# DorianaG01/trajectory_generation

Measured on AMD Instinct MI355X. Metric: MPC steps/sec (batch=4096, N=20), higher is better.
Workload: dtype f64

## Files before the change

### trajectory_generation_amd/csrc/mpc_common.h

```cpp
#pragma once
#include "physics.h"

#ifndef TGMPC_DPP_BC
#define TGMPC_DPP_BC 0
#endif

namespace tgmpc {

constexpr double INFTY = 1e30;
constexpr double DIV_TOL = 1e-30;
constexpr double MIN_SCALING = 1e-4;
constexpr double MAX_SCALING = 1e4;
constexpr double RHO_MIN = 1e-6;
constexpr double RHO_MAX = 1e6;
constexpr double RHO_TOL = 1e-4;
constexpr double RHO_EQ_OVER_INEQ = 1e3;

struct PathArgs {
    int kmax;
    const int* kind;
    const double* pc;
    const int* nk;
    const double* xk;
    const double* coef;
};

#define TRAJ_FUSED_MAX_PER_WG 8

struct KArgs {
    traj_vehicle_params p;
    traj_mpc_config c;
    int B;
    const double* x0;
    const double* u_prev;
    const double* path_ref;
    const double* vref;
    const double* Ad;
    const double* Bd;
    const double* gd;
    double* u_cmd;
    int* status;
    double* objective;
    double* X_opt;
    double* U_opt;
    int* iters;
    int* polished;
    PathArgs path;
    double* x_state;
    double* u_state;
    int t, hist_T;
    double* hist_x;
    double* hist_u;
    long long* dbg;
    double* wsA;
    double* wsB;
    double* wsg;
    double* wsXF;
    double* wsWarm;
    const int* perm;
    int nsteps;
    int fused_grid;
    int* queue;
    int spin_limit;
    long long* dbg_items;
    int lead_steps, lead_h;
    int run_ahead;
    int wps;
};

__device__ __forceinline__ void st_coh(double* p, double v) {
    __hip_atomic_store(p, v, __ATOMIC_RELAXED, __HIP_MEMORY_SCOPE_AGENT);
}
__device__ __forceinline__ double ld_coh(const double* p) {
    return __hip_atomic_load(const_cast<double*>(p), __ATOMIC_RELAXED, __HIP_MEMORY_SCOPE_AGENT);
}

__device__ __forceinline__ double limit_scaling(double v) {
    return v < MIN_SCALING ? 1.0 : (v > MAX_SCALING ? MAX_SCALING : v);
}

__device__ inline void path_eval(const PathArgs& pa, int b, double x, double& y, double& dy) {
    int kind = pa.kind[b];
    const double* c = pa.pc + 4 * b;
    if (kind == 0) {
        y = c[0] + x * (c[1] + x * (c[2] + x * c[3]));
        dy = c[1] + x * (2.0 * c[2] + x * 3.0 * c[3]);
    } else if (kind == 1) {
        double a = c[1] * x + c[2];
        double s, co;
        pm_sincos(a, &s, &co);
        y = c[0] * s + c[3];
        dy = c[0] * c[1] * co;
    } else {
        int nk = pa.nk[b];
        const double* xk = pa.xk + (size_t)pa.kmax * b;
        const double* cf = pa.coef + (size_t)(pa.kmax - 1) * 4 * b;
        if (x <= xk[0]) {
            y = cf[0] + cf[1] * (x - xk[0]);
            dy = cf[1];
        } else if (x >= xk[nk - 1]) {
            const double* q = cf + 4 * (nk - 2);
            double h = xk[nk - 1] - xk[nk - 2];
            double ye = q[0] + h * (q[1] + h * (q[2] + h * q[3]));
            double se = q[1] + h * (2.0 * q[2] + h * 3.0 * q[3]);
            y = ye + se * (x - xk[nk - 1]);
            dy = se;
        } else {
            int j = 0;
            while (j < nk - 2 && x >= xk[j + 1]) ++j;
            const double* q = cf + 4 * j;
            double tt = x - xk[j];
            y = q[0] + tt * (q[1] + tt * (q[2] + tt * q[3]));
            dy = q[1] + tt * (2.0 * q[2] + tt * 3.0 * q[3]);
        }
    }
}

template <int V>
__device__ __forceinline__ void wave_max(double (&v)[V]) {
#pragma unroll
    for (int off = 32; off >= 1; off >>= 1) {
#pragma unroll
        for (int i = 0; i < V; ++i) {
            double o = __shfl_xor(v[i], off, 64);
            v[i] = (o > v[i] || o != o) ? o : v[i];
        }
    }
}

__device__ __forceinline__ double uniformize(double v) {
    const long long bits = __double_as_longlong(v);
    const int lo = __builtin_amdgcn_readfirstlane((int)(bits & 0xffffffffLL));
    const int hi = __builtin_amdgcn_readfirstlane((int)(bits >> 32));
    return __longlong_as_double(((long long)hi << 32) | (unsigned int)lo);
}

__device__ __forceinline__ double wave_sum(double v) {
#pragma unroll
    for (int off = 32; off >= 1; off >>= 1) v += __shfl_xor(v, off, 64);
    return v;
}

__device__ __forceinline__ double rcp_nr(double d) {
    double r = __builtin_amdgcn_rcp(d);
    r = fma(fma(-d, r, 1.0), r, r);
    r = fma(fma(-d, r, 1.0), r, r);
    return r;
}

__device__ __forceinline__ double vmax(double a, double b) {
    double r;
    asm("v_max_f64 %0, %1, %2" : "=v"(r) : "v"(a), "v"(b));
    return r;
}
__device__ __forceinline__ double vmin(double a, double b) {
    double r;
    asm("v_min_f64 %0, %1, %2" : "=v"(r) : "v"(a), "v"(b));
    return r;
}
__device__ __forceinline__ double clamp_mm(double x, double lo, double hi) { return vmin(vmax(x, lo), hi); }
__device__ __forceinline__ double vmax_abs(double a, double b) {
    double r;
    asm("v_max_f64 %0, %1, |%2|" : "=v"(r) : "v"(a), "v"(b));
    return r;
}
__device__ __forceinline__ double vmax_abs2(double a, double b) {
    double r;
    asm("v_max_f64 %0, |%1|, |%2|" : "=v"(r) : "v"(a), "v"(b));
    return r;
}

__device__ __forceinline__ unsigned opaque_u(unsigned v) {
    asm volatile("" : "+v"(v));
    return v;
}
__device__ __forceinline__ double bitsel(unsigned m, double a, double b) {
    const unsigned long long ua = __double_as_longlong(a), ub = __double_as_longlong(b);
    const unsigned lo = (unsigned(ua) & m) | (unsigned(ub) & ~m);
    const unsigned hi = (unsigned(ua >> 32) & m) | (unsigned(ub >> 32) & ~m);
    return __longlong_as_double((long long)(((unsigned long long)hi << 32) | lo));
}

__device__ __forceinline__ double sqrt_n(double x) {
    const double y = __builtin_amdgcn_rsq(x);
    double g = x * y, h = y * 0.5;
    const double r = fma(-h, g, 0.5);
    g = fma(g, r, g);
    const double d0 = fma(-g, g, x);
    h = fma(h, r, h);
    g = fma(d0, h, g);
    const double d1 = fma(-g, g, x);
    return fma(d1, h, g);
}
__device__ __forceinline__ double rcp_n(double b) {
    double y = __builtin_amdgcn_rcp(b);
    double e = fma(-b, y, 1.0);
    y = fma(y, e, y);
    e = fma(-b, y, 1.0);
    y = fma(y, e, y);
    const double r = fma(-b, y, 1.0);
    return fma(r, y, y);
}

__device__ __forceinline__ double cdiv(double d, double c, double y) {
    double q = d * y, t, r;
    asm("v_fma_f64 %0, %1, %2, -%3" : "=v"(t) : "v"(q), "v"(c), "v"(d));
    asm("v_fma_f64 %0, -%1, %2, %3" : "=v"(r) : "v"(t), "v"(y), "v"(q));
    return r;
}

__device__ __forceinline__ double fma3(double a, double b, double c) {
    double r;
    asm("v_fma_f64 %0, %1, %2, %3" : "=v"(r) : "v"(a), "v"(b), "v"(c));
    return r;
}

__device__ __forceinline__ double fma3n(double a, double b, double c) {
    double r;
    asm("v_fma_f64 %0, -%1, %2, %3" : "=v"(r) : "v"(a), "v"(b), "v"(c));
    return r;
}

template <int NN>
__device__ __forceinline__ void lds_load_all(const double* p, double (&o)[NN]) {
    const double2* p2 = reinterpret_cast<const double2*>(__builtin_assume_aligned(p, 16));
#pragma unroll
    for (int i = 0; i < NN / 2; ++i) {
        const double2 v = p2[i];
        o[2 * i] = v.x;
        o[2 * i + 1] = v.y;
    }
    __builtin_amdgcn_sched_group_barrier(0x100, NN / 2, 0);
}

typedef double v2d_t __attribute__((ext_vector_type(2)));
template <int OFF>
__device__ __forceinline__ void lds_load10_masked(unsigned a, unsigned long long m, v2d_t* r) {
    unsigned long long sv;
    asm volatile(
        "s_mov_b64 %[sv], exec\n\t"
        "s_and_b64 exec, exec, %[m]\n\t"
        "ds_read_b128 %[r0], %[a] offset:%[o0]\n\t"
        "ds_read_b128 %[r1], %[a] offset:%[o1]\n\t"
        "ds_read_b128 %[r2], %[a] offset:%[o2]\n\t"
        "ds_read_b128 %[r3], %[a] offset:%[o3]\n\t"
        "ds_read_b128 %[r4], %[a] offset:%[o4]\n\t"
        "ds_read_b128 %[r5], %[a] offset:%[o5]\n\t"
        "ds_read_b128 %[r6], %[a] offset:%[o6]\n\t"
        "ds_read_b128 %[r7], %[a] offset:%[o7]\n\t"
        "ds_read_b128 %[r8], %[a] offset:%[o8]\n\t"
        "ds_read_b128 %[r9], %[a] offset:%[o9]\n\t"
        "s_waitcnt lgkmcnt(0)\n\t"
        "s_mov_b64 exec, %[sv]"
        : [sv] "=&s"(sv), [r0] "+v"(r[0]), [r1] "+v"(r[1]), [r2] "+v"(r[2]), [r3] "+v"(r[3]), [r4] "+v"(r[4]), [r5] "+v"(r[5]), [r6] "+v"(r[6]), [r7] "+v"(r[7]), [r8] "+v"(r[8]), [r9] "+v"(r[9])
        : [a] "v"(a), [m] "s"(m), [o0] "i"(OFF + 0), [o1] "i"(OFF + 16), [o2] "i"(OFF + 32), [o3] "i"(OFF + 48), [o4] "i"(OFF + 64), [o5] "i"(OFF + 80), [o6] "i"(OFF + 96), [o7] "i"(OFF + 112), [o8] "i"(OFF + 128), [o9] "i"(OFF + 144)
        : "memory");
}

template <int CTRL, int ROW_MASK = 0xf>
__device__ __forceinline__ double dpp_d(double v) {
    int lo = __double2loint(v), hi = __double2hiint(v);
#if TGMPC_DPP_BC
    if constexpr (ROW_MASK == 0xf) {
        lo = __builtin_amdgcn_mov_dpp(lo, CTRL, 0xf, 0xf, true);
        hi = __builtin_amdgcn_mov_dpp(hi, CTRL, 0xf, 0xf, true);
        return __hiloint2double(hi, lo);
    }
#endif
    lo = __builtin_amdgcn_update_dpp(0, lo, CTRL, ROW_MASK, 0xf, false);
    hi = __builtin_amdgcn_update_dpp(0, hi, CTRL, ROW_MASK, 0xf, false);
    return __hiloint2double(hi, lo);
}
__device__ __forceinline__ double lane_up2(double v) { return dpp_d<0x130>(dpp_d<0x130>(v)); }
__device__ __forceinline__ double lane_dn2(double v) { return dpp_d<0x138>(dpp_d<0x138>(v)); }

__device__ __forceinline__ double readlane_d(double v, int l) {
    int lo = __builtin_amdgcn_readlane(__double2loint(v), l);
    int hi = __builtin_amdgcn_readlane(__double2hiint(v), l);
    return __hiloint2double(hi, lo);
}

template <int V>
__device__ __forceinline__ void wave_max_dpp(double (&v)[V]) {
#pragma unroll
    for (int i = 0; i < V; ++i) {
        const bool nan = __ballot(v[i] != v[i]) != 0;
        double m = v[i];
        m = vmax(m, dpp_d<0xB1>(m));
        m = vmax(m, dpp_d<0x4E>(m));
        m = vmax(m, dpp_d<0x141>(m));
        m = vmax(m, dpp_d<0x140>(m));
        m = vmax(m, dpp_d<0x142, 0xa>(m));
        m = vmax(m, dpp_d<0x143, 0xc>(m));
        m = readlane_d(m, 63);
        v[i] = nan ? __builtin_nan("") : m;
    }
}

__device__ __forceinline__ double wave_sum_dpp(double v) {
    v += dpp_d<0xB1>(v);
    v += dpp_d<0x4E>(v);
    v += dpp_d<0x141>(v);
    v += dpp_d<0x140>(v);
    v += dpp_d<0x142, 0xa>(v);
    v += dpp_d<0x143, 0xc>(v);
    return readlane_d(v, 63);
}


}
```

### trajectory_generation_amd/csrc/mpc_linearize.h

```cpp
#pragma once
#include "mpc_common.h"

namespace tgmpc {

constexpr double DQ_INV = 1.0 / (2.0 * 1e-5);

__device__ __forceinline__ void rollout_f(const VP& p, const double* x, double d, double delta, double sd, double cd,
                                          double* xd) {
    const double phi = x[2], vx = x[3], vy = x[4], omega = x[5];
    const double avx = fabs(vx);
    const double mx = (p.vx_zero > avx) ? p.vx_zero : avx;
    const double vx_eff = np_sign(vx) * mx;
    const double alpha_f = clampd(-pm_atan2(omega * p.lf + vy, vx_eff) + delta, -p.maxAlpha, p.maxAlpha);
    const double alpha_r = clampd(pm_atan2(omega * p.lr - vy, vx_eff), -p.maxAlpha, p.maxAlpha);
    double sphi, cphi;
    const double sf = pm_tire_sin(p.Cf * pm_atan(p.Bf * alpha_f));
    const double sr = pm_tire_sin(p.Cr * pm_atan(p.Br * alpha_r));
    pm_sincos(phi, &sphi, &cphi);
    const double Fy_f = p.Df * sf, Fy_r = p.Dr * sr;
    const double Frx = (p.Cm1 - p.Cm2 * vx) * d - p.Cr0 - p.Cr2 * (vx * vx);
    xd[0] = vx * cphi - vy * sphi;
    xd[1] = vx * sphi + vy * cphi;
    xd[2] = omega;
    xd[3] = (1.0 / p.m) * (Frx - Fy_f * sd + p.m * vy * omega);
    xd[4] = (1.0 / p.m) * (Fy_r + Fy_f * cd - p.m * vx * omega);
    xd[5] = (1.0 / p.Iz) * (Fy_f * p.lf * cd - Fy_r * p.lr);
}

template <bool CLOSED>
__global__ __launch_bounds__(64) void rollout_kernel(const KArgs a) {
    const int b = blockIdx.x * 64 + threadIdx.x;
    if (b >= a.B) return;
    const traj_vehicle_params& p = a.p;
    const int N = a.c.N;
    const double Ts = a.c.Ts;
    const double* xs = CLOSED ? a.x_state + 6 * (size_t)b : a.x0 + 6 * (size_t)b;
    const double* us = CLOSED ? a.u_state + 2 * (size_t)b : a.u_prev + 2 * (size_t)b;
    double x[6], f[6];
    for (int i = 0; i < 6; ++i) x[i] = xs[i];
    const double u0 = us[0], u1 = us[1];
    double sd, cd;
    pm_sincos(u1, &sd, &cd);
    double* rec = a.wsXF + (size_t)b * N * 12;
    for (int k = 0; k < N; ++k) {
        rollout_f(p, x, u0, u1, sd, cd, f);
        for (int i = 0; i < 6; ++i) {
            rec[12 * k + i] = x[i];
            rec[12 * k + 6 + i] = f[i];
            x[i] = x[i] + Ts * f[i];
        }
    }
}

struct Tire {
    double vx_eff, atf, atr;
};
__device__ __forceinline__ Tire tire_angles(const VP& p, double vx, double vy, double omega) {
    Tire r;
    const double avx = fabs(vx);
    const double mx = (p.vx_zero > avx) ? p.vx_zero : avx;
    r.vx_eff = np_sign(vx) * mx;
    r.atf = pm_atan2(omega * p.lf + vy, r.vx_eff);
    r.atr = pm_atan2(omega * p.lr - vy, r.vx_eff);
    return r;
}
__device__ __forceinline__ double tire_sin(double z) { return pm_tire_sin(z); }
__device__ __forceinline__ double front_force(const VP& p, double atf, double delta) {
    const double alpha_f = clampd(-atf + delta, -p.maxAlpha, p.maxAlpha);
    return p.Df * tire_sin(p.Cf * pm_atan(p.Bf * alpha_f));
}
__device__ __forceinline__ double rear_force(const VP& p, double atr) {
    const double alpha_r = clampd(atr, -p.maxAlpha, p.maxAlpha);
    return p.Dr * tire_sin(p.Cr * pm_atan(p.Br * alpha_r));
}
__device__ __forceinline__ double long_force(const VP& p, double vx, double d) {
    return (p.Cm1 - p.Cm2 * vx) * d - p.Cr0 - p.Cr2 * (vx * vx);
}
__device__ __forceinline__ void f_parts(const VP& p, double vx, double vy, double omega, double sphi, double cphi,
                                        double sd, double cd, double Fy_f, double Fy_r, double Frx, double* xd) {
    xd[0] = vx * cphi - vy * sphi;
    xd[1] = vx * sphi + vy * cphi;
    xd[2] = omega;
    xd[3] = (1.0 / p.m) * (Frx - Fy_f * sd + p.m * vy * omega);
    xd[4] = (1.0 / p.m) * (Fy_r + Fy_f * cd - p.m * vx * omega);
    xd[5] = (1.0 / p.Iz) * (Fy_f * p.lf * cd - Fy_r * p.lr);
}
__device__ __forceinline__ void f_full(const VP& p, double vx, double vy, double omega, double sphi, double cphi,
                                       double d, double delta, double sd, double cd, double* xd) {
    const Tire tr = tire_angles(p, vx, vy, omega);
    f_parts(p, vx, vy, omega, sphi, cphi, sd, cd, front_force(p, tr.atf, delta), rear_force(p, tr.atr),
            long_force(p, vx, d), xd);
}

__device__ __forceinline__ void state_column(const VP& p, const double* xb, double d, double de, int grp, double* J) {
    const double eps = 1e-5;
    const double phi = xb[2] + 0.0, vx = xb[3] + 0.0, vy = xb[4] + 0.0, om = xb[5] + 0.0;
    double sphi, cphi, sd, cd;
    pm_sincos(phi, &sphi, &cphi);
    pm_sincos(de, &sd, &cd);
    double fp[6], fm[6];
    f_full(p, grp == 0 ? xb[3] + eps : vx, grp == 1 ? xb[4] + eps : vy, grp == 2 ? xb[5] + eps : om, sphi, cphi, d,
           de, sd, cd, fp);
    f_full(p, grp == 0 ? xb[3] - eps : vx, grp == 1 ? xb[4] - eps : vy, grp == 2 ? xb[5] - eps : om, sphi, cphi, d,
           de, sd, cd, fm);
    for (int r = 0; r < 6; ++r) J[r] = cdiv(fp[r] - fm[r], 2.0 * eps, DQ_INV);
}

__device__ __forceinline__ void cheap_columns(const VP& p, const double* xb, double d, double de, double* Jphi,
                                              double* Jd, double* Jde) {
    const double eps = 1e-5;
    const double phi = xb[2] + 0.0, vx = xb[3] + 0.0, vy = xb[4] + 0.0, om = xb[5] + 0.0;
    double sphi, cphi, sd, cd;
    pm_sincos(phi, &sphi, &cphi);
    pm_sincos(de, &sd, &cd);
    double fp[6], fm[6];
    const Tire t0 = tire_angles(p, vx, vy, om);
    const double Ff0 = front_force(p, t0.atf, de), Fr0 = rear_force(p, t0.atr), Fx0 = long_force(p, vx, d);
    {
        double sp, cp, sm, cm;
        pm_sincos(xb[2] + eps, &sp, &cp);
        pm_sincos(xb[2] - eps, &sm, &cm);
        f_parts(p, vx, vy, om, sp, cp, sd, cd, Ff0, Fr0, Fx0, fp);
        f_parts(p, vx, vy, om, sm, cm, sd, cd, Ff0, Fr0, Fx0, fm);
        for (int r = 0; r < 6; ++r) Jphi[r] = cdiv(fp[r] - fm[r], 2.0 * eps, DQ_INV);
    }
    {
        f_parts(p, vx, vy, om, sphi, cphi, sd, cd, Ff0, Fr0, long_force(p, vx, d + eps), fp);
        f_parts(p, vx, vy, om, sphi, cphi, sd, cd, Ff0, Fr0, long_force(p, vx, d - eps), fm);
        for (int r = 0; r < 6; ++r) Jd[r] = cdiv(fp[r] - fm[r], 2.0 * eps, DQ_INV);
    }
    {
        double sp, cp, sm, cm;
        pm_sincos(de + eps, &sp, &cp);
        pm_sincos(de - eps, &sm, &cm);
        f_parts(p, vx, vy, om, sphi, cphi, sp, cp, front_force(p, t0.atf, de + eps), Fr0, Fx0, fp);
        f_parts(p, vx, vy, om, sphi, cphi, sm, cm, front_force(p, t0.atf, de - eps), Fr0, Fx0, fm);
        for (int r = 0; r < 6; ++r) Jde[r] = cdiv(fp[r] - fm[r], 2.0 * eps, DQ_INV);
    }
    if ((__builtin_signbit(xb[2]) && xb[2] == 0.0) || (__builtin_signbit(xb[3]) && xb[3] == 0.0) ||
        (__builtin_signbit(xb[4]) && xb[4] == 0.0) || (__builtin_signbit(xb[5]) && xb[5] == 0.0) ||
        (__builtin_signbit(d) && d == 0.0) || (__builtin_signbit(de) && de == 0.0)) {
        for (int cu = 0; cu < 2; ++cu) {
            const double up[2] = {cu == 0 ? d + eps : d + 0.0, cu == 1 ? de + eps : de + 0.0};
            const double um[2] = {cu == 0 ? d - eps : d + 0.0, cu == 1 ? de - eps : de + 0.0};
            double xc[6];
            for (int i = 0; i < 6; ++i) xc[i] = xb[i];
            f_cont(p, xc, up, fp);
            f_cont(p, xc, um, fm);
            for (int r = 0; r < 6; ++r) (cu == 0 ? Jd : Jde)[r] = cdiv(fp[r] - fm[r], 2.0 * eps, DQ_INV);
        }
    }
}

__device__ __forceinline__ double a_entry(int r, int cc, double Ts, double Jrc) {
    return ((r == cc) ? 1.0 : 0.0) + Ts * Jrc;
}
__device__ __forceinline__ void g_stage(const double* A, const double* Bm, const double* xb, const double* fk, double d,
                                       double de, double Ts, double* g) {
    for (int r = 0; r < 6; ++r) {
        double ax = 0.0, bu = 0.0;
        for (int cc = 0; cc < 6; ++cc) ax += A[6 * r + cc] * xb[cc];
        bu += Bm[2 * r] * d;
        bu += Bm[2 * r + 1] * de;
        g[r] = xb[r] + Ts * fk[r] - ax - bu;
    }
}

template <bool CLOSED>
__global__ __launch_bounds__(256) void jac_kernel(const KArgs a) {
    __shared__ double sJ[64][6][6];
    const int N = a.c.N;
    const int s = threadIdx.x & 63, grp = threadIdx.x >> 6;
    const int gs = blockIdx.x * 64 + s;
    const bool valid = gs < a.B * N;
    const int b = valid ? gs / N : 0, k = valid ? gs - b * N : 0;
    const traj_vehicle_params& p = a.p;
    const double Ts = a.c.Ts;
    const double* rec = a.wsXF + ((size_t)b * N + k) * 12;
    const double* us = CLOSED ? a.u_state + 2 * (size_t)b : a.u_prev + 2 * (size_t)b;
    double xb[6];
    for (int i = 0; i < 6; ++i) xb[i] = valid ? rec[i] : 0.0;
    const double d = valid ? us[0] : 0.0, de = valid ? us[1] : 0.0;
    double (*J)[6] = sJ[s];
    if (grp < 3) state_column(p, xb, d, de, grp, J[1 + grp]);
    else cheap_columns(p, xb, d, de, J[0], J[4], J[5]);
    __syncthreads();
    if (grp != 3 || !valid) return;
    double A[36], Bm[12], g[6];
    for (int r = 0; r < 6; ++r) {
        A[6 * r + 0] = a_entry(r, 0, Ts, 0.0);
        A[6 * r + 1] = a_entry(r, 1, Ts, 0.0);
        for (int cc = 2; cc < 6; ++cc) A[6 * r + cc] = a_entry(r, cc, Ts, J[cc - 2][r]);
        Bm[2 * r + 0] = Ts * J[4][r];
        Bm[2 * r + 1] = Ts * J[5][r];
    }
    g_stage(A, Bm, xb, rec + 6, d, de, Ts, g);
    const size_t o = (size_t)b * N + k;
    double* wA = a.wsA + o * 36;
    double* wB = a.wsB + o * 12;
    double* wg = a.wsg + o * 6;
    for (int i = 0; i < 36; ++i) wA[i] = A[i];
    for (int i = 0; i < 12; ++i) wB[i] = Bm[i];
    for (int r = 0; r < 6; ++r) wg[r] = g[r];
}

constexpr int TJ = 24;
constexpr int LREC = 54;
static_assert(TJ + 12 <= 36, "a stage's scratch must lie inside its record's A_k part");
template <int NT>
__device__ __forceinline__ void block_linearize(const int t, const VP& p, int N, double Ts, const double* xs,
                                                const double* us, double* rec, long long* dbg = nullptr) {
    double* const tj = rec;
    double* const xf = rec + TJ;
    auto mark = [&](int i) { if (dbg && t == 0) dbg[i] = __builtin_amdgcn_s_memtime(); };
    const double eps = 1e-5;
    if (t < 64) {
        double x[6];
        for (int i = 2; i < 6; ++i) x[i] = xs[i];
        const double u0 = us[0], u1 = us[1];
        double sd, cd;
        pm_sincos(u1, &sd, &cd);
        const bool roll = t < 2;
        const bool fr = (t == 0) || (t == 3) || (t >= 5 && t <= 16 && ((t - 5) & 1) == 0) || t == 17 || t == 18;
        const int col = (t >= 5 && t <= 16) ? (t - 5) >> 2 : -1;
        const double sgn = (t >= 5 && t <= 16 && ((t - 5) & 2)) ? -eps : eps;
        const double dlt = (t == 17) ? u1 + eps : ((t == 18) ? u1 - eps : u1);
        const double Bt = fr ? p.Bf : p.Br, Ct = fr ? p.Cf : p.Cr;
        const double dvx = roll ? -0.0 : (col == 0 ? sgn : 0.0);
        const double dvy = roll ? -0.0 : (col == 1 ? sgn : 0.0);
        const double dom = roll ? -0.0 : (col == 2 ? sgn : 0.0);
        const double Lt = fr ? p.lf : p.lr, sy = fr ? 1.0 : -1.0, sa = fr ? -1.0 : 1.0, dl = fr ? dlt : -0.0;
        const unsigned long long used = 0x7fffbull;
        for (int k = 0; k < N; ++k) {
            const double phi = x[2], vx = x[3], vy = x[4], omega = x[5];
            const double vxl = vx + dvx, vyl = vy + dvy, oml = omega + dom;
            const double avx = fabs(vxl);
            const double mx = (p.vx_zero > avx) ? p.vx_zero : avx;
            const double vx_eff = np_sign(vxl) * mx;
            const double at = pm_atan2(oml * Lt + sy * vyl, vx_eff);
            const double alpha = clampd(sa * at + dl, -p.maxAlpha, p.maxAlpha);
            const double z = Ct * pm_atan(Bt * alpha);
            double sz = tire_sin_poly(z);
            if (__ballot(!tire_sin_in_range(z)) & used) {
                if (!tire_sin_in_range(z)) sz = pm_sin(z);
            }
            if (t >= 3 && t <= 18) tj[LREC * k + t] = sz;
            const double Fy_f = p.Df * readlane_d(sz, 0), Fy_r = p.Dr * readlane_d(sz, 1);
            const double Frx = (p.Cm1 - p.Cm2 * vx) * u0 - p.Cr0 - p.Cr2 * (vx * vx);
            double f[6];
            f[2] = omega;
            f[3] = (1.0 / p.m) * (Frx - Fy_f * sd + p.m * vy * omega);
            f[4] = (1.0 / p.m) * (Fy_r + Fy_f * cd - p.m * vx * omega);
            f[5] = (1.0 / p.Iz) * (Fy_f * p.lf * cd - Fy_r * p.lr);
            if (t == 0)
                for (int i = 2; i < 6; ++i) {
                    xf[LREC * k + i] = x[i];
                    xf[LREC * k + 6 + i] = f[i];
                }
            for (int i = 2; i < 6; ++i) x[i] = x[i] + Ts * f[i];
            (void)phi;
        }
    }
    __syncthreads();
    for (int l = t; l < 3 * N; l += NT) {
        const int v = l / N, k = l - v * N;
        const double phik = xf[LREC * k + 2];
        double sp, cp;
        pm_sincos(phik + (v == 0 ? -0.0 : (v == 1 ? eps : -eps)), &sp, &cp);
        double* const T = tj + LREC * k;
        if (v == 0) {
            T[21] = sp + 0.0;
            T[2] = cp;
            const double vx = xf[LREC * k + 3], vy = xf[LREC * k + 4];
            xf[LREC * k + 6] = vx * cp - vy * sp;
            xf[LREC * k + 7] = vx * sp + vy * cp;
        } else {
            T[18 + v] = sp;
            T[v - 1] = cp;
        }
    }
    __syncthreads();
    if (t == 0) {
        double X = xs[0], Y = xs[1];
        for (int k = 0; k < N; ++k) {
            xf[LREC * k + 0] = X;
            xf[LREC * k + 1] = Y;
            X = X + Ts * xf[LREC * k + 6];
            Y = Y + Ts * xf[LREC * k + 7];
        }
    }
    __syncthreads();
    mark(20);
    mark(21);
    const double d = us[0], de = us[1];
    double sd, cd, sdp, cdp, sdm, cdm;
    pm_sincos(de, &sd, &cd);
    pm_sincos(de + eps, &sdp, &cdp);
    pm_sincos(de - eps, &sdm, &cdm);
    for (int k = t; k < N; k += NT) {
        const double* T = tj + LREC * k;
        double xb[6], fk[6];
        for (int i = 0; i < 6; ++i) { xb[i] = xf[LREC * k + i]; fk[i] = xf[LREC * k + 6 + i]; }
        const double vx0 = xb[3] + 0.0, vy0 = xb[4] + 0.0, om0 = xb[5] + 0.0;
        const double sphi = T[21], cphi = T[2];
        const double Ff0 = p.Df * T[3], Fr0 = p.Dr * T[4], Fx0 = long_force(p, vx0, d);
        double Ak[36], Bk[12], fp[6], fm[6];
        for (int grp = 0; grp < 3; ++grp) {
            const double vxp = grp == 0 ? xb[3] + eps : vx0, vxm = grp == 0 ? xb[3] - eps : vx0;
            const double vyp = grp == 1 ? xb[4] + eps : vy0, vym = grp == 1 ? xb[4] - eps : vy0;
            const double omp = grp == 2 ? xb[5] + eps : om0, omm = grp == 2 ? xb[5] - eps : om0;
            const int l = 5 + 4 * grp;
            f_parts(p, vxp, vyp, omp, sphi, cphi, sd, cd, p.Df * T[l], p.Dr * T[l + 1], long_force(p, vxp, d), fp);
            f_parts(p, vxm, vym, omm, sphi, cphi, sd, cd, p.Df * T[l + 2], p.Dr * T[l + 3], long_force(p, vxm, d), fm);
            for (int r = 0; r < 6; ++r) Ak[6 * r + 3 + grp] = a_entry(r, 3 + grp, Ts, cdiv(fp[r] - fm[r], 2.0 * eps, DQ_INV));
        }
        double Jphi[6], Jd[6], Jde[6];
        f_parts(p, vx0, vy0, om0, T[19], T[0], sd, cd, Ff0, Fr0, Fx0, fp);
        f_parts(p, vx0, vy0, om0, T[20], T[1], sd, cd, Ff0, Fr0, Fx0, fm);
        for (int r = 0; r < 6; ++r) Jphi[r] = cdiv(fp[r] - fm[r], 2.0 * eps, DQ_INV);
        f_parts(p, vx0, vy0, om0, sphi, cphi, sd, cd, Ff0, Fr0, long_force(p, vx0, d + eps), fp);
        f_parts(p, vx0, vy0, om0, sphi, cphi, sd, cd, Ff0, Fr0, long_force(p, vx0, d - eps), fm);
        for (int r = 0; r < 6; ++r) Jd[r] = cdiv(fp[r] - fm[r], 2.0 * eps, DQ_INV);
        f_parts(p, vx0, vy0, om0, sphi, cphi, sdp, cdp, p.Df * T[17], Fr0, Fx0, fp);
        f_parts(p, vx0, vy0, om0, sphi, cphi, sdm, cdm, p.Df * T[18], Fr0, Fx0, fm);
        for (int r = 0; r < 6; ++r) Jde[r] = cdiv(fp[r] - fm[r], 2.0 * eps, DQ_INV);
        if ((__builtin_signbit(xb[2]) && xb[2] == 0.0) || (__builtin_signbit(xb[3]) && xb[3] == 0.0) ||
            (__builtin_signbit(xb[4]) && xb[4] == 0.0) || (__builtin_signbit(xb[5]) && xb[5] == 0.0) ||
            (__builtin_signbit(d) && d == 0.0) || (__builtin_signbit(de) && de == 0.0)) {
            for (int cu = 0; cu < 2; ++cu) {
                const double up[2] = {cu == 0 ? d + eps : d + 0.0, cu == 1 ? de + eps : de + 0.0};
                const double um[2] = {cu == 0 ? d - eps : d + 0.0, cu == 1 ? de - eps : de + 0.0};
                double xc[6];
                for (int i = 0; i < 6; ++i) xc[i] = xb[i];
                f_cont(p, xc, up, fp);
                f_cont(p, xc, um, fm);
                for (int r = 0; r < 6; ++r) (cu == 0 ? Jd : Jde)[r] = cdiv(fp[r] - fm[r], 2.0 * eps, DQ_INV);
            }
        }
        for (int r = 0; r < 6; ++r) {
            Ak[6 * r + 0] = a_entry(r, 0, Ts, 0.0);
            Ak[6 * r + 1] = a_entry(r, 1, Ts, 0.0);
            Ak[6 * r + 2] = a_entry(r, 2, Ts, Jphi[r]);
            Bk[2 * r + 0] = Ts * Jd[r];
            Bk[2 * r + 1] = Ts * Jde[r];
        }
        double gk[6];
        g_stage(Ak, Bk, xb, fk, d, de, Ts, gk);
        double* const o = rec + LREC * k;
        for (int i = 0; i < 36; ++i) o[i] = Ak[i];
        for (int i = 0; i < 12; ++i) o[36 + i] = Bk[i];
        for (int r = 0; r < 6; ++r) o[48 + r] = gk[r];
    }
    __syncthreads();
}

}
```

### trajectory_generation_amd/csrc/physics.h

```cpp
#pragma once
#include <hip/hip_runtime.h>

#include "../../include/trajmpc.h"
#include "fastmath.h"

#ifndef TGMPC_FASTMATH
#define TGMPC_FASTMATH 0
#endif

namespace tgmpc {

__device__ __forceinline__ void pm_sincos(double x, double* s, double* c) {
#if TGMPC_FASTMATH
    fm_sincos(x, s, c);
#else
    sincos(x, s, c);
#endif
}
__device__ __forceinline__ double pm_sin(double x) {
    double s, c;
    pm_sincos(x, &s, &c);
    return s;
}
__device__ __forceinline__ double pm_atan(double x) {
#if TGMPC_FASTMATH
    return fm_atan(x);
#else
    return atan(x);
#endif
}
__device__ __forceinline__ double pm_atan2(double y, double x) {
#if TGMPC_FASTMATH
    return fm_atan2(y, x);
#else
    return atan2(y, x);
#endif
}

typedef traj_vehicle_params VP;

constexpr double TIRE_SIN_ZMAX = 1.5707963267948966;
__device__ __forceinline__ double tire_sin_poly(double x) {
    const double x2 = x * x;
    double q = 1.9572941063391263e-20;
    q = fma(q, x2, -8.22063524662433e-18);
    q = fma(q, x2, 2.8114572543455206e-15);
    q = fma(q, x2, -7.647163731819816e-13);
    q = fma(q, x2, 1.6059043836821613e-10);
    q = fma(q, x2, -2.505210838544172e-08);
    q = fma(q, x2, 2.7557319223985893e-06);
    q = fma(q, x2, -0.0001984126984126984);
    q = fma(q, x2, 0.008333333333333333);
    q = fma(q, x2, -0.16666666666666666);
    return fma(x2 * x, q, x);
}
__device__ __forceinline__ bool tire_sin_in_range(double z) { return fabs(z) <= TIRE_SIN_ZMAX; }
__device__ __forceinline__ double pm_tire_sin(double z) {
    return tire_sin_in_range(z) ? tire_sin_poly(z) : pm_sin(z);
}

__device__ __forceinline__ double np_sign(double x) {
    return x > 0.0 ? 1.0 : (x < 0.0 ? -1.0 : (x == 0.0 ? 0.0 : x));
}

__device__ __forceinline__ double clampd(double x, double lo, double hi) {
    double t = (x < lo) ? lo : x;
    return (t > hi) ? hi : t;
}

__device__ __forceinline__ void tire_forces(const VP& p, double vx, double vy, double omega, double d, double delta,
                                            double& Fy_f, double& Fy_r, double& Frx) {
    double avx = fabs(vx);
    double mx = (p.vx_zero > avx) ? p.vx_zero : avx;
    double vx_eff = np_sign(vx) * mx;
    double alpha_f = -pm_atan2(omega * p.lf + vy, vx_eff) + delta;
    double alpha_r = pm_atan2(omega * p.lr - vy, vx_eff);
    alpha_f = clampd(alpha_f, -p.maxAlpha, p.maxAlpha);
    alpha_r = clampd(alpha_r, -p.maxAlpha, p.maxAlpha);
    Fy_f = p.Df * pm_tire_sin(p.Cf * pm_atan(p.Bf * alpha_f));
    Fy_r = p.Dr * pm_tire_sin(p.Cr * pm_atan(p.Br * alpha_r));
    Frx = (p.Cm1 - p.Cm2 * vx) * d - p.Cr0 - p.Cr2 * (vx * vx);
}

__device__ __forceinline__ void f_cont_sc(const VP& p, const double* x, double d, double delta, double sd, double cd,
                                          double* xd) {
    double phi = x[2], vx = x[3], vy = x[4], omega = x[5];
    double Fy_f, Fy_r, Frx;
    tire_forces(p, vx, vy, omega, d, delta, Fy_f, Fy_r, Frx);
    double sphi, cphi;
    pm_sincos(phi, &sphi, &cphi);
    xd[0] = vx * cphi - vy * sphi;
    xd[1] = vx * sphi + vy * cphi;
    xd[2] = omega;
    xd[3] = (1.0 / p.m) * (Frx - Fy_f * sd + p.m * vy * omega);
    xd[4] = (1.0 / p.m) * (Fy_r + Fy_f * cd - p.m * vx * omega);
    xd[5] = (1.0 / p.Iz) * (Fy_f * p.lf * cd - Fy_r * p.lr);
}

__device__ __forceinline__ void f_cont(const VP& p, const double* x, const double* u, double* xd) {
    double sd, cd;
    pm_sincos(u[1], &sd, &cd);
    f_cont_sc(p, x, u[0], u[1], sd, cd, xd);
}

__device__ __forceinline__ double lateral_error(double X, double Y, double Xr, double Yr, double phir) {
    double s, c;
    pm_sincos(phir, &s, &c);
    return s * (X - Xr) - c * (Y - Yr);
}

}
```

Baseline: 17.04 million.

## Add lean inline atan/atan2 fast path in linearize rollout with guarded fallback

```diff
diff --git a/trajectory_generation_amd/csrc/mpc_common.h b/trajectory_generation_amd/csrc/mpc_common.h
--- a/trajectory_generation_amd/csrc/mpc_common.h
+++ b/trajectory_generation_amd/csrc/mpc_common.h
@@ -202,6 +202,17 @@
     return fma(r, y, y);
 }
 
+__device__ __forceinline__ double div_n(double a, double b) {
+    double y = __builtin_amdgcn_rcp(b);
+    double e = fma(-b, y, 1.0);
+    y = fma(y, e, y);
+    e = fma(-b, y, 1.0);
+    y = fma(y, e, y);
+    const double q = a * y;
+    const double r = fma(-b, q, a);
+    return fma(r, y, q);
+}
+
 __device__ __forceinline__ double cdiv(double d, double c, double y) {
     double q = d * y, t, r;
     asm("v_fma_f64 %0, %1, %2, -%3" : "=v"(t) : "v"(q), "v"(c), "v"(d));
@@ -219,6 +230,71 @@
     double r;
     asm("v_fma_f64 %0, -%1, %2, %3" : "=v"(r) : "v"(a), "v"(b), "v"(c));
     return r;
+}
+
+
+__device__ __forceinline__ double fma3s(double a, double b, double c) {
+    double r;
+    asm("v_fma_f64 %0, %1, %2, %3" : "=v"(r) : "v"(a), "v"(b), "s"(c));
+    return r;
+}
+__device__ __forceinline__ double vmax_s(double c, double b) {
+    double r;
+    asm("v_max_f64 %0, %1, %2" : "=v"(r) : "s"(c), "v"(b));
+    return r;
+}
+__device__ __forceinline__ double vmin_s(double a, double c) {
+    double r;
+    asm("v_min_f64 %0, %1, %2" : "=v"(r) : "v"(a), "s"(c));
+    return r;
+}
+__device__ __forceinline__ double vmax_sneg(double a, double c) {
+    double r;
+    asm("v_max_f64 %0, %1, -%2" : "=v"(r) : "v"(a), "s"(c));
+    return r;
+}
+__device__ __forceinline__ double vmin_abs(double a, double b) {
+    double r;
+    asm("v_min_f64 %0, %1, |%2|" : "=v"(r) : "v"(a), "v"(b));
+    return r;
+}
+
+__device__ __forceinline__ double atanred_n(double v) {
+    constexpr unsigned long long C[20] = {
+        0x3EEBA404B5E68A13ull, 0xBF23E260BD3237F4ull, 0x3F4B2BB069EFB384ull, 0xBF67952DAF56DE9Bull,
+        0x3F7D6D43A595C56Full, 0xBF8C6EA4A57D9582ull, 0x3F967E295F08B19Full, 0xBF9E9AE6FC27006Aull,
+        0x3FA2C15B5711927Aull, 0xBFA59976E82D3FF0ull, 0x3FA82D5D6EF28734ull, 0xBFAAE5CE6A214619ull,
+        0x3FAE1BB48427B883ull, 0xBFB110E48B207F05ull, 0x3FB3B13657B87036ull, 0xBFB745D119378E4Full,
+        0x3FBC71C717E1913Cull, 0xBFC2492492376B7Dull, 0x3FC99999999952CCull, 0xBFD5555555555523ull};
+    const double t = v * v;
+    double z = fma(t, __builtin_bit_cast(double, C[0]), __builtin_bit_cast(double, C[1]));
+#pragma unroll
+    for (int i = 2; i < 20; ++i) z = fma(t, z, __builtin_bit_cast(double, C[i]));
+    return fma(v, t * z, v);
+}
+
+__device__ __forceinline__ double atan2_n(double y, double x) {
+    const double u = vmax_abs(x, y), v = vmin_abs(x, y);
+    const double a = atanred_n(div_n(v, u));
+    const double s = __builtin_bit_cast(double, 0x3FF921FB54442D18ull) - a;
+    return copysign((x < fabs(y)) ? s : a, y);
+}
+
+__device__ __forceinline__ double atan_n(double x) {
+    const double ax = fabs(x);
+    const bool g = ax > 1.0;
+    const double a = atanred_n(g ? rcp_n(ax) : ax);
+    const double c = fma(__builtin_bit_cast(double, 0x3FEDD9AD336A0500ull),
+                         __builtin_bit_cast(double, 0x3FFAF154EEB562D6ull), -a);
+    return copysign(g ? c : a, x);
+}
+
+__device__ __forceinline__ double tire_sin_poly_s(double x) {
+    const double x2 = x * x;
+    double q = fma(TIRE_SIN_Q[0], x2, TIRE_SIN_Q[1]);
+#pragma unroll
+    for (int i = 2; i < 10; ++i) q = fma3s(q, x2, TIRE_SIN_Q[i]);
+    return fma(x2 * x, q, x);
 }
 
 template <int NN>
diff --git a/trajectory_generation_amd/csrc/mpc_linearize.h b/trajectory_generation_amd/csrc/mpc_linearize.h
--- a/trajectory_generation_amd/csrc/mpc_linearize.h
+++ b/trajectory_generation_amd/csrc/mpc_linearize.h
@@ -214,12 +214,14 @@
     double* const xf = rec + TJ;
     auto mark = [&](int i) { if (dbg && t == 0) dbg[i] = __builtin_amdgcn_s_memtime(); };
     const double eps = 1e-5;
+    const int ln = t & 63;
+    double s_de, c_de;
+    pm_sincos(ln == 1 ? us[1] + eps : (ln == 2 ? us[1] - eps : us[1]), &s_de, &c_de);
     if (t < 64) {
         double x[6];
         for (int i = 2; i < 6; ++i) x[i] = xs[i];
         const double u0 = us[0], u1 = us[1];
-        double sd, cd;
-        pm_sincos(u1, &sd, &cd);
+        const double sd = readlane_d(s_de, 0), cd = readlane_d(c_de, 0);
         const bool roll = t < 2;
         const bool fr = (t == 0) || (t == 3) || (t >= 5 && t <= 16 && ((t - 5) & 1) == 0) || t == 17 || t == 18;
         const int col = (t >= 5 && t <= 16) ? (t - 5) >> 2 : -1;
@@ -231,16 +233,29 @@
         const double dom = roll ? -0.0 : (col == 2 ? sgn : 0.0);
         const double Lt = fr ? p.lf : p.lr, sy = fr ? 1.0 : -1.0, sa = fr ? -1.0 : 1.0, dl = fr ? dlt : -0.0;
         const unsigned long long used = 0x7fffbull;
+        constexpr unsigned LEAN_LO = 0x33700000u, LEAN_HI = 0x4C700000u;
+        const bool lean_item = !TGMPC_FASTMATH && p.vx_zero >= 0x1p-200 && p.vx_zero <= 0x1p200 &&
+                               p.maxAlpha > 0.0 && fabs(u1) < 0x1p99 && fabs(Bt) < 0x1p100;
         for (int k = 0; k < N; ++k) {
             const double phi = x[2], vx = x[3], vy = x[4], omega = x[5];
             const double vxl = vx + dvx, vyl = vy + dvy, oml = omega + dom;
-            const double avx = fabs(vxl);
-            const double mx = (p.vx_zero > avx) ? p.vx_zero : avx;
-            const double vx_eff = np_sign(vxl) * mx;
-            const double at = pm_atan2(oml * Lt + sy * vyl, vx_eff);
-            const double alpha = clampd(sa * at + dl, -p.maxAlpha, p.maxAlpha);
-            const double z = Ct * pm_atan(Bt * alpha);
-            double sz = tire_sin_poly(z);
+            const double yt = oml * Lt + sy * vyl;
+            const unsigned hx = (unsigned)__double2hiint(vxl), hy = (unsigned)__double2hiint(yt) & 0x7fffffffu;
+            const bool in_dom = lean_item && (hx - 1u < LEAN_HI - 1u) &&
+                                ((hy - LEAN_LO < LEAN_HI - LEAN_LO) || yt == 0.0);
+            const double at_n = atan2_n(yt, vmax_s(p.vx_zero, vxl));
+            const double w = Bt * vmin_s(vmax_sneg(sa * at_n + dl, p.maxAlpha), p.maxAlpha);
+            double z = Ct * atan_n(w);
+            double sz = tire_sin_poly_s(z);
+            if (__builtin_amdgcn_ballot_w64(!in_dom) & used) {
+                const double avx = fabs(vxl);
+                const double mx = (p.vx_zero > avx) ? p.vx_zero : avx;
+                const double vx_eff = np_sign(vxl) * mx;
+                const double at = pm_atan2(yt, vx_eff);
+                const double alpha = clampd(sa * at + dl, -p.maxAlpha, p.maxAlpha);
+                z = Ct * pm_atan(Bt * alpha);
+                sz = tire_sin_poly(z);
+            }
             if (__ballot(!tire_sin_in_range(z)) & used) {
                 if (!tire_sin_in_range(z)) sz = pm_sin(z);
             }
@@ -293,10 +308,9 @@
     mark(20);
     mark(21);
     const double d = us[0], de = us[1];
-    double sd, cd, sdp, cdp, sdm, cdm;
-    pm_sincos(de, &sd, &cd);
-    pm_sincos(de + eps, &sdp, &cdp);
-    pm_sincos(de - eps, &sdm, &cdm);
+    const double sd = readlane_d(s_de, 0), cd = readlane_d(c_de, 0);
+    const double sdp = readlane_d(s_de, 1), cdp = readlane_d(c_de, 1);
+    const double sdm = readlane_d(s_de, 2), cdm = readlane_d(c_de, 2);
     for (int k = t; k < N; k += NT) {
         const double* T = tj + LREC * k;
         double xb[6], fk[6];
diff --git a/trajectory_generation_amd/csrc/physics.h b/trajectory_generation_amd/csrc/physics.h
--- a/trajectory_generation_amd/csrc/physics.h
+++ b/trajectory_generation_amd/csrc/physics.h
@@ -40,18 +40,15 @@
 typedef traj_vehicle_params VP;
 
 constexpr double TIRE_SIN_ZMAX = 1.5707963267948966;
+constexpr double TIRE_SIN_Q[10] = {1.9572941063391263e-20, -8.22063524662433e-18,  2.8114572543455206e-15,
+                                   -7.647163731819816e-13, 1.6059043836821613e-10, -2.505210838544172e-08,
+                                   2.7557319223985893e-06, -0.0001984126984126984, 0.008333333333333333,
+                                   -0.16666666666666666};
 __device__ __forceinline__ double tire_sin_poly(double x) {
     const double x2 = x * x;
-    double q = 1.9572941063391263e-20;
-    q = fma(q, x2, -8.22063524662433e-18);
-    q = fma(q, x2, 2.8114572543455206e-15);
-    q = fma(q, x2, -7.647163731819816e-13);
-    q = fma(q, x2, 1.6059043836821613e-10);
-    q = fma(q, x2, -2.505210838544172e-08);
-    q = fma(q, x2, 2.7557319223985893e-06);
-    q = fma(q, x2, -0.0001984126984126984);
-    q = fma(q, x2, 0.008333333333333333);
-    q = fma(q, x2, -0.16666666666666666);
+    double q = TIRE_SIN_Q[0];
+#pragma unroll
+    for (int i = 1; i < 10; ++i) q = fma(q, x2, TIRE_SIN_Q[i]);
     return fma(x2 * x, q, x);
 }
 __device__ __forceinline__ bool tire_sin_in_range(double z) { return fabs(z) <= TIRE_SIN_ZMAX; }
```

Measured after the change: 17.13 million (median of 6 runs). About the same (+0.5%).
